# austinjeng/Shift-GCN

Measured on AMD Instinct MI355X. Metric: skeleton clips/sec fwd+bwd, NTU (3,300,25,2) bs=64; 1/2/4/8 MI355X, higher is better.
Workload: dtype fp32; 1 GPU; NTU Shift-GCN training step (fwd+CE+bwd+SGD), x=(64,3,300,25,2) per GPU; global_batch=64, per_gpu_batch=64, parallelism=dp1, hipgraph=False, world_size=1, backend=none

## Files before the change

### include/shiftgcn.h

```cpp
#ifndef SHIFTGCN_H_
#define SHIFTGCN_H_

#include <stddef.h>

#ifdef __cplusplus
extern "C" {
#endif

#define SGCN_EINVAL (-22)
#define SGCN_ABI_VERSION 25
#define SGCN_ABI_DIAG_FLAG 0x10000

int sgcn_abi_version(void);


int sgcn_tshift_fwd(const float* in, float* out, const float* xpos, const float* ypos,
                    const float* in_scale, const float* in_shift, float* plane_stats,
                    int B, int C, int H, int W, int stride, int ypos_is_raw, void* stream);

int sgcn_tshift_fwd_pre(const float* z, float* out, const float* xpos, const float* ypos,
                        const float* pre_scale, const float* pre_shift, const float* r,
                        const float* r_scale, const float* r_shift, const float* in_scale,
                        const float* in_shift, int B, int C, int H, int W, int stride,
                        int ypos_is_raw, void* stream);
// ... 92 lines not shown
                         const float* mean, const float* invstd, const float* gamma,
                         float* dgamma, float* dbeta, int accumulate, int batch_stats,
                         float* coef, void* stream);

int sgcn_bn_bwd_finalize_gbn(const float* part6, int B, int C, int V, long long n_total,
                             const float* dy_coef, const float* dy_mean, const float* mean,
                             const float* invstd, const float* gamma, float* dgamma,
                             float* dbeta, int accumulate, int batch_stats, float* coef,
                             void* stream);

int sgcn_bn_bwd_apply(const float* dy, const float* y, int relu, const float* x,
                      const float* coef, int per_joint, const float* r, const float* rcoef,
                      const float* dy_coef, float* dx, float* dr, int B, int C, int T, int V,
                      void* stream);

int sgcn_mask_prep(const float* mask, float* m, int n, void* stream);

int sgcn_gcn_gather(const float* x0, const float* m, float* xg, int B, int C, int T, int V,
                    void* stream);

#define SGCN_DXF_MASK_DX 1
#define SGCN_DXF_ADD2_PLANE 2
int sgcn_gcn_dx_finish(const float* dxt, const float* x0, const float* m, const float* add1,
                       const float* add2, const float* add2_mask, float* dx, float* dmask_part,
                       const float* prev_s, const float* prev_mean, const float* prev_invstd,
                       float* prev_part, int B, int C, int T, int V, int flags, void* stream);

int sgcn_mask_grad_finalize(const float* part, const float* mask, int B, int C, int V,
                            float* dmask, int accumulate, void* stream);

// ... 67 lines not shown
```

### shift-gcn_amd/csrc/bn.hip

```cpp
#include "common.hpp"
#include "dispatch.hpp"
#include "launch_forms.hpp"

namespace sgcn {
namespace {

constexpr int kU = 4;

constexpr int kUM = 8;

template <bool PER_JOINT, bool ZU = false>
__global__ __launch_bounds__(kThreads) void moments_kernel(const float* __restrict__ x,
                                                            float2* __restrict__ part, int T,
                                                            int V, int C) {
  SGCN_CRIT_PRIO();
  __shared__ float s1[kThreads], s2[kThreads], red[2 * kThreads / 64];
  const int plane = gridDim.x - 1 - blockIdx.x;
  const int P = T * V;
  const float* __restrict__ xp = x + (size_t)plane * P;
  const int i = threadIdx.x;
  if (PER_JOINT) {
    const int G = kThreads / V;
    float a = 0.f, q = 0.f;
    const int v = i % V, r = i / V;
// ... 730 lines not shown
  const int f = PER_JOINT ? c * V + w : c;
  const float k1 = coef[f], k2 = coef[F + f], k3 = coef[2 * F + f];
  float d1 = 1.f, d2 = 0.f, d3 = 0.f, q1 = 0.f, q2 = 0.f, q3 = 0.f;
  if (DYT) { d1 = dyc[c]; d2 = dyc[C + c]; d3 = dyc[2 * C + c]; }
  if (RES == 2) { q1 = rcoef[c]; q2 = rcoef[RF + c]; q3 = rcoef[2 * RF + c]; }
  const auto dxr = make_rsrc(dx + off, pb);
  const auto drr = make_rsrc(RES ? dr + off : dx + off, RES ? pb : 0u);
#pragma unroll
  for (int e = 0; e < LPT; ++e) {
    float g = gv[e];
    if (DYT) g = d1 * g + d2 * yv[e] + d3;
    if (RELU) g = yv[e] > 0.f ? g : 0.f;
    bstore(dxr, k1 * g + k2 * xv[e] + k3, go + e * vstep, 0);
    if (RES == 1) bstore(drr, g, vo + e * vstep, 0);
    if (RES == 2) bstore(drr, q1 * g + q2 * rv[e] + q3, vo + e * vstep, 0);
  }
}

template <int NT, int LPT, bool ADD1, bool ADD2, bool PART, int A2M>
__global__ __launch_bounds__(NT) void gcn_dx_finish_ja_kernel(
    const float* __restrict__ dxt, const float* __restrict__ x0, const float* __restrict__ m,
    const float* __restrict__ add1, const float* __restrict__ add2, float* __restrict__ dx,
    float* __restrict__ dmask_part, const float* __restrict__ ps,
    const float* __restrict__ pmean, const float* __restrict__ pinvstd,
    float2* __restrict__ bn_part, int C, int T, int V, const float* __restrict__ add2m,
    int flags) {
  SGCN_CRIT_PRIO();
  __shared__ float s0[NT];
  __shared__ float red[2 * NT / 64];
  const int plane = blockIdx.x, c = plane % C, rc = c % V;
// ... 427 lines not shown
    bn_bwd_apply_ja_kernel<NT, LPT, PJM, RL, RS, DYT><<<g, int(NT), 0, st>>>(
        dy, y, x, coef, F, r, rcoef, C, dy_coef, dx, dr, C, T, V);
  };
  auto loop = [&](auto PJM, auto RL, auto RS, auto DYT) {
    bn_bwd_apply_kernel<PJM, RL, RS, DYT><<<g, kThreads, 0, st>>>(
        dy, y, x, coef, F, r, rcoef, C, dy_coef, dx, dr, C, T, V);
  };
  const bool ok = per_joint == 3
                      ? launch_plane(T, V, ja, loop, Const<3>{}, Const<true>{}, rs, dyt)
                      : launch_plane(T, V, ja, loop, Const<0>{}, relu != 0, rs, dyt);
  SGCN_REQUIRE(ok);
  SGCN_LAUNCH_CHECK();
  return 0;
}

int sgcn_mask_prep(const float* mask, float* m, int n, void* stream) {
  SGCN_REQUIRE(mask && m && n > 0);
  mask_prep_kernel<<<(n + 255) / 256, 256, 0, (hipStream_t)stream>>>(mask, m, n);
  SGCN_LAUNCH_CHECK();
  return 0;
}

int sgcn_mask_prep_many(const float* const* mask, float* const* m, const int* count, int n,
                        void* stream) {
  SGCN_REQUIRE(n >= 0 && n <= SGCN_BATCH_MAX);
  if (n == 0) return 0;
  SGCN_REQUIRE(mask && m && count);
  MaskPrepBatch t{};
  int mx = 0;
  for (int i = 0; i < n; ++i) {
// ... 90 lines not shown
```

### shift-gcn_amd/csrc/tshift.hip

```cpp
#include "common.hpp"
#include "dispatch.hpp"
#include "launch_forms.hpp"

#pragma clang fp contract(off)

namespace sgcn {
namespace {


struct Geom {
  int x1, y1;
  float dx, dy;
};

__device__ __forceinline__ Geom make_geom(float x, float y) {
  Geom g;
  g.x1 = (int)floorf(x);
  g.y1 = (int)floorf(y);
  g.dx = x - (float)g.x1;
  g.dy = y - (float)g.y1;
  return g;
}

__device__ __forceinline__ float blend(float q11, float q21, float q12, float q22, float dx,
                                       float dy) {
  const float omdx = 1.f - dx, omdy = 1.f - dy;
  return q11 * omdx * omdy + q21 * dx * omdy + q12 * omdx * dy + q22 * dx * dy;
}

struct Walker {
  int h, w, dh, dw, W;
  __device__ __forceinline__ Walker(int o0, int step, int W_) : W(W_) {
    h = o0 / W_;
    w = o0 - h * W_;
    dh = step / W_;
    dw = step - dh * W_;
  }
  __device__ __forceinline__ void next() {
    h += dh;
    w += dw;
    if (w >= W) { w -= W; ++h; }
  }
};
// ... 204 lines not shown
          const float gg = o < nt ? gv[e] : 0.f;
          ax += vx * gg;
          ay += vy * gg;
        }
      }
    }
  }
  block_sum2(ax, ay, red);
  if (threadIdx.x == 0) pgrad[plane] = make_float2(ax, ay);
  if (BNP) {
    block_sum2(bs0, bs1, red);
    if (threadIdx.x == 0) bn_part[plane] = make_float2(bs0, bs1);
  }
}


template <int NT>
__device__ __forceinline__ void zero_pad(float* lds, int H, int W) {
  const int WP = W + 2, nprow = 2 * kPadRows * WP;
  for (int i = (int)threadIdx.x; i < nprow + 2 * H; i += NT) {
    int a;
    if (i < nprow) {
      const int r = i / WP, col = i - r * WP;
      a = (r < kPadRows ? r : H + r) * WP + col;
    } else {
      const int j = i - nprow;
      a = ((j >> 1) + kPadRows) * WP + ((j & 1) ? W + 1 : 0);
    }
    lds[a] = 0.f;
  }
}

template <int NT, int LPT, bool AFFINE>
__device__ __forceinline__ void stage_plane(const float* __restrict__ src, float* lds, int n,
                                            float a, float b) {
  float t[LPT];
#pragma unroll
  for (int e = 0; e < LPT; ++e) t[e] = src[min(e * NT + (int)threadIdx.x, n - 1)];
#pragma unroll
  for (int e = 0; e < LPT; ++e) {
    const int i = e * NT + threadIdx.x;
    if (i < n) lds[i] = AFFINE ? t[e] * a + b : t[e];
  }
}

template <int NT, int EPT, int LPT, bool AFFINE, bool STATS>
// ... 453 lines not shown
    }
  }
  if (BNP) {
    block_sum4(ax, ay, bs0, bs1, red);
    if (threadIdx.x == 0) {
      pgrad[plane] = make_float2(ax, ay);
      bn_part[plane] = make_float2(bs0, bs1);
    }
  } else {
    block_sum2(ax, ay, red);
    if (threadIdx.x == 0) pgrad[plane] = make_float2(ax, ay);
  }
}

template <int NT, int LPT, bool AFFINE, bool RELU_MASK, bool BNP, int GP, bool GBN,
          bool GBD = false>
__global__ __launch_bounds__(NT) void tshift_bwd_ra_kernel(
    const float* __restrict__ gout, const float* __restrict__ in,
    const float* __restrict__ xpos, const float* __restrict__ ypos,
    const float* __restrict__ scale, const float* __restrict__ shift,
    const float* __restrict__ bn_mean, const float* __restrict__ bn_invstd,
    float* __restrict__ gin, float2* __restrict__ pgrad, float2* __restrict__ bn_part, int C,
    int H, int W, const float* __restrict__ gdy, const float* __restrict__ gy,
    const float* __restrict__ gx, const float* __restrict__ gcoef,
    const float* __restrict__ gz, const float* __restrict__ gzm,
    const float* __restrict__ gzi, float* __restrict__ gzpart, const float* __restrict__ gd = nullptr,
    const float* __restrict__ gdm = nullptr, const float* __restrict__ gdi = nullptr,
    float* __restrict__ gdpart = nullptr, int gdyp = 0) {
  SGCN_CRIT_PRIO();
  static_assert(!GBN || (AFFINE && BNP && !GP), "GBN: shift_in with BNP");
  static_assert(!GBD || GBN, "GBD extends GBN");
  extern __shared__ float lds[];
  __shared__ float red[4 * NT / 64];
  const int plane = gridDim.x - 1 - blockIdx.x;
  const int c = plane % C;
  const int n = H * W, WP = W + 2;
  const int GR = NT / W, NTE = GR * W;
  const int tid = threadIdx.x;
  const bool own = tid < NTE;
  const int w = tid % W, h0 = tid / W;
  const unsigned vo = own ? (unsigned)tid * 4u : 0x80000000u;
  const unsigned vstep = (unsigned)NTE * 4u, nbytes = (unsigned)n * 4u;
  const size_t poff = (size_t)plane * n;
  float t[LPT], rin_r[LPT];
  float zr[GBN ? LPT : 1], dr[GBD ? LPT : 1];
  {
// ... 57 lines not shown
    lds[own && e * NTE + tid < n ? lbase + e * lstep : lspare] = t[e];
  float bmu = 0.f, bis = 0.f;
  if (BNP) { bmu = bn_mean[c]; bis = bn_invstd[c]; }
  const float x = xpos[c], y = ypos[c];
  float a = 1.f, b = 0.f;
  if (AFFINE) { a = scale[c]; b = shift[c]; }
  float zm = 0.f, zi = 0.f, dmu = 0.f, dis = 0.f;
  if (GBN) { zm = gzm[c * W + w]; zi = gzi[c * W + w]; }
  if (GBD) { dmu = gdm[c]; dis = gdi[c]; }
  __syncthreads();

  const Geom r = make_geom(-x, -y);
  const Geom g = make_geom(x, y);
  const bool fits = r.y1 >= -kPadRows && r.y1 <= kPadRows - 1 && g.y1 >= -kPadRows &&
                    g.y1 <= kPadRows - 1 && r.x1 >= -1 && r.x1 <= 0 && g.x1 >= -1 && g.x1 <= 0;
  const int kq = r.y1 * WP + r.x1, kg = (-g.y1 - 1) * WP - g.x1 - 1;
  const int nfull = n / NTE;
  const int lmax = (H - 1 + kPadRows) * WP + W;
  const auto gir = make_rsrc(gin + poff, nbytes);
  float bs0 = 0.f, bs1 = 0.f, ax = 0.f, ay = 0.f;
  float a6[6] = {0.f, 0.f, 0.f, 0.f, 0.f, 0.f};
  float d6[6] = {0.f, 0.f, 0.f, 0.f, 0.f, 0.f};
  auto elem = [&](int e, bool tail, float q11, float q21, float q12, float q22, float G11,
                  float G21, float G12, float G22) {
    const bool ok = !tail || e * NTE + tid < n;
    float val = blend(q11, q21, q12, q22, r.dx, r.dy);
    const float rin = rin_r[e];
    if (RELU_MASK) val = rin > 0.f ? val : 0.f;
    if (tail) val = ok ? val : 0.f;
    bstore(gir, val, vo + e * vstep, 0);
    if (GBN) {
      const bool act = rin > 0.f;
      const float hc = act ? rin - bmu : 0.f, zh = act ? (zr[e] - zm) * zi : 0.f;
      const float vv = act ? val : 0.f;
      a6[0] += vv;
      a6[1] += hc;
      a6[2] += act ? 1.f : 0.f;
      a6[3] = fmaf(vv, zh, a6[3]);
      a6[4] = fmaf(hc, zh, a6[4]);
      a6[5] += zh;
      if (GBD) {
        const float dh = act ? (dr[e] - dmu) * dis : 0.f;
        d6[0] += vv;
        d6[1] += hc;
        d6[2] += act ? 1.f : 0.f;
// ... 7 lines not shown
      bs1 = fmaf(val, (rin - bmu) * bis, bs1);
    }
    const float cx = (1.f - g.dy) * (G21 - G11) + g.dy * (G22 - G12);
    const float cy = (1.f - g.dx) * (G12 - G11) + g.dx * (G22 - G21);
    float qa = AFFINE ? rin * a + b : rin;
    if (tail) qa = ok ? qa : 0.f;
    ax = fmaf(qa, cx, ax);
    ay = fmaf(qa, cy, ay);
  };
  if (own && fits) {
    int l0 = lbase;
#pragma unroll
    for (int e = 0; e < LPT; ++e) {
      const bool tail = e >= nfull;
      const int lt = min(l0, lmax);
      const int la = lt + kq, lg = lt + kg;
      elem(e, tail, lds[la], lds[la + 1], lds[la + WP], lds[la + WP + 1], lds[lg + WP + 1],
           lds[lg + WP], lds[lg + 1], lds[lg]);
      l0 += lstep;
      asm volatile("" : "+v"(l0));
    }
  } else if (own) {
    const auto inr = make_rsrc(in + poff, nbytes);
    const auto zrr = make_rsrc(GBN ? gz + poff : in + poff, nbytes);
    int wz = w - c % W;
    wz = wz < 0 ? wz + W : wz;
    auto tap = [&](int row, int col) {
      const bool in_ = (unsigned)row < (unsigned)H && (unsigned)col < (unsigned)W;
      const int rr = min(max(row, 0), H - 1), cc = min(max(col, 0), W - 1);
      const float v = lds[(rr + kPadRows) * WP + cc + 1];
      return in_ ? v : 0.f;
    };
#pragma unroll 1
    for (int e = 0; e < LPT; ++e) {
      const int h = h0 + e * GR;
      const bool ok = e * NTE + tid < n;
      const float rin = bload(inr, vo + e * vstep, 0);
      const float zv = GBN ? bload(zrr, vo + e * vstep + (unsigned)((wz - w) * 4), 0) : 0.f;
      const int rq = h + r.y1, cq = w + r.x1, rg = h - g.y1 - 1, cg = w - g.x1 - 1;
      float val = blend(tap(rq, cq), tap(rq, cq + 1), tap(rq + 1, cq), tap(rq + 1, cq + 1),
                        r.dx, r.dy);
      if (RELU_MASK) val = rin > 0.f ? val : 0.f;
      val = ok ? val : 0.f;
      bstore(gir, val, vo + e * vstep, 0);
      if (GBN && rin > 0.f) {
        const float hc = rin - bmu, zh = (zv - zm) * zi;
        a6[0] += val;
        a6[1] += hc;
        a6[2] += 1.f;
        a6[3] = fmaf(val, zh, a6[3]);
        a6[4] = fmaf(hc, zh, a6[4]);
        a6[5] += zh;
        if (GBD) {
          const float dh = (bload(make_rsrc(gd + poff, nbytes), vo + e * vstep, 0) - dmu) * dis;
          d6[0] += val;
          d6[1] += hc;
          d6[2] += 1.f;
          d6[3] = fmaf(val, dh, d6[3]);
          d6[4] = fmaf(hc, dh, d6[4]);
// ... 117 lines not shown
  const float *gout, *in, *xpos, *ypos, *scale, *shift, *bmu, *bis;
  float* gin;
  float2 *pg, *bp;
  int B, C, H, W;
  const float *gdy, *gy, *gx, *gcoef;
  int gdyp;
  const float *gz, *gzm, *gzi;
  float* gzpart;
  const float *gd, *gdm, *gdi;
  float* gdpart;
};

template <const auto& Forms, class... A>
bool launch_ra(const LaunchForm& f, const RaArgs& a, hipStream_t st, A... flags) {
  return with_form<Forms>({f.nt, f.lpt}, [&](auto NT, auto LPT, auto AFFINE, auto RELU, auto BNP,
                                           auto GP, auto GBN, auto GBD) {
    tshift_bwd_ra_kernel<NT, LPT, AFFINE, RELU, BNP, GP, GBN, GBD>
        <<<a.B * a.C, int(NT), ra_lds_bytes(a.H, a.W, NT, GBN), st>>>(
            a.gout, a.in, a.xpos, a.ypos, a.scale, a.shift, a.bmu, a.bis, a.gin, a.pg, a.bp, a.C,
            a.H, a.W, a.gdy, a.gy, a.gx, a.gcoef, a.gz, a.gzm, a.gzi, a.gzpart, a.gd, a.gdm,
            a.gdi, a.gdpart, a.gdyp);
  }, flags...);
}

}
}

using namespace sgcn;

extern "C" {

int sgcn_tshift_fwd(const float* in, float* out, const float* xpos, const float* ypos,
// ... 120 lines not shown
  SGCN_REQUIRE(f.kind == Kind::ra);
  SGCN_REQUIRE(dy && s && coef && in && xpos && ypos && gin && ws);
  SGCN_REQUIRE((gx == nullptr) == (gy == nullptr));
  SGCN_REQUIRE(ws_bytes >= sgcn_tshift_bwd_ws_bytes(B, C));
  SGCN_REQUIRE((long long)B * C < (1LL << 31));
  (void)ypos_is_raw;
  hipStream_t st = (hipStream_t)stream;
  float2* pg = (float2*)ws;
  RaArgs a{nullptr, in, xpos, ypos, nullptr, nullptr, nullptr, nullptr, gin, pg, nullptr, B, C, H, W};
  a.gdy = dy;
  a.gy = y;
  a.gx = s;
  a.gcoef = coef;
  a.gdyp = dy_plane != 0;
  const bool ok = launch_ra<kBninForms>(f, a, st, Const<false>{}, Const<true>{}, Const<false>{},
                                        OneOf<1, 2>{y ? 1 : 2}, Const<false>{}, Const<false>{});
  SGCN_REQUIRE(ok);
  SGCN_LAUNCH_CHECK();
  if (gx) tshift_pos_finalize_kernel<<<(C + 3) / 4, 256, 0, st>>>(pg, B, C, gx, gy);
  SGCN_LAUNCH_CHECK();
  return 0;
}

size_t sgcn_tshift_bwd_ws_bytes(int B, int C) { return (size_t)B * C * sizeof(float2); }

int sgcn_tshift_pos_finalize_many(const void* const* partials, float* const* gx,
                                  float* const* gy, const int* B, const int* C, int n,
                                  void* stream) {
  SGCN_REQUIRE(n >= 0 && n <= SGCN_BATCH_MAX);
  if (n == 0) return 0;
  SGCN_REQUIRE(partials && gx && gy && B && C);
// ... 21 lines not shown
  return 0;
}

int sgcn_tshift_bwd_gbn(const float* gout, const float* in, const float* xpos,
                        const float* ypos, const float* in_scale, const float* in_shift,
                        const float* bn_mean, const float* bn_invstd, float* bn_part,
                        const float* z, const float* z_mean, const float* z_invstd,
                        float* z_part, const float* d, const float* d_mean,
                        const float* d_invstd, float* d_part, float* gin, float* gx, float* gy,
                        void* ws, size_t ws_bytes, int B, int C, int H, int W, void* stream) {
  SGCN_REQUIRE(B > 0 && C > 0 && H > 0 && W > 0);
  SGCN_REQUIRE((d == nullptr) == (d_part == nullptr) && (!d || (d_mean && d_invstd)));
  const LaunchForm f = gbn_form(H, W, d != nullptr);
  SGCN_REQUIRE(f.kind == Kind::ra);
  SGCN_REQUIRE(gout && in && xpos && ypos && in_scale && in_shift && bn_mean && bn_invstd &&
               bn_part && z && z_mean && z_invstd && z_part && gin && ws);
  SGCN_REQUIRE((gx == nullptr) == (gy == nullptr));
  SGCN_REQUIRE(ws_bytes >= sgcn_tshift_bwd_ws_bytes(B, C));
  SGCN_REQUIRE((long long)B * C < (1LL << 31));
  hipStream_t st = (hipStream_t)stream;
  float2* pg = (float2*)ws;
  RaArgs a{gout, in, xpos, ypos, in_scale, in_shift, bn_mean, bn_invstd, gin, pg,
           (float2*)bn_part, B, C, H, W};
  a.gz = z;
  a.gzm = z_mean;
  a.gzi = z_invstd;
  a.gzpart = z_part;
  if (d) {
    a.gd = d;
    a.gdm = d_mean;
    a.gdi = d_invstd;
    a.gdpart = d_part;
  }
  const Const<true> on{};
  const Const<false> off{};
  const bool ok = d ? launch_ra<kGbdForms>(f, a, st, on, off, on, Const<0>{}, on, on)
                    : launch_ra<kRaForms>(f, a, st, on, off, on, Const<0>{}, on, off);
  SGCN_REQUIRE(ok);
  SGCN_LAUNCH_CHECK();
  if (gx) tshift_pos_finalize_kernel<<<(C + 3) / 4, 256, 0, st>>>(pg, B, C, gx, gy);
  SGCN_LAUNCH_CHECK();
  return 0;
}

int sgcn_tshift_bwd(const float* gout, const float* in, const float* xpos, const float* ypos,
                    const float* in_scale, const float* in_shift, int relu_mask,
                    const float* bn_mean, const float* bn_invstd, float* bn_part, float* gin,
                    float* gx, float* gy, void* ws, size_t ws_bytes, int B, int C, int H,
                    int W, int stride, int ypos_is_raw, void* stream) {
  SGCN_REQUIRE(B > 0 && C > 0 && H >= 0 && W > 0 && (stride == 1 || stride == 2));
  SGCN_REQUIRE((in_scale == nullptr) == (in_shift == nullptr));
  const int Ho = H / stride;
  SGCN_REQUIRE((gout || Ho == 0) && (in || H == 0) && (gin || H == 0));
  SGCN_REQUIRE(xpos && ypos && ws && (gx == nullptr) == (gy == nullptr));
  SGCN_REQUIRE(!bn_part || (bn_mean && bn_invstd));
  SGCN_REQUIRE(ws_bytes >= sgcn_tshift_bwd_ws_bytes(B, C));
  SGCN_REQUIRE((long long)H * W < (1LL << 30) && (long long)B * C < (1LL << 31));
  hipStream_t st = (hipStream_t)stream;
  const bool aff = in_scale != nullptr, relu = relu_mask != 0, bnp = bn_part != nullptr;
  float2* pg = (float2*)ws;
  float2* bp = (float2*)bn_part;
  const int ah = (ypos_is_raw && stride != 1) ? 1 : 0;
  const LaunchForm f = bwd_form(H, W, stride);
  bool ok;
  if (f.kind == Kind::ra) {
    const RaArgs a{gout, in, xpos, ypos, in_scale, in_shift, bn_mean, bn_invstd, gin, pg, bp, B,
                   C, H, W};
    ok = launch_ra<kRaForms>(f, a, st, aff, relu, bnp, Const<0>{}, Const<false>{}, Const<false>{});
  } else if (f.kind == Kind::s2) {
    const size_t lds = (size_t)(H + Ho) * W * sizeof(float);
    ok = with_consts([&](auto LPT, auto JA, auto AFFINE, auto RELU, auto BNP) {
      tshift_bwd_s2_kernel<kBwdThreads, LPT, AFFINE, RELU, BNP, JA><<<B * C, kBwdThreads, lds, st>>>(
          gout, in, xpos, ypos, in_scale, in_shift, bn_mean, bn_invstd, gin, pg, bp, C, H, W, Ho,
          ah);
    }, OneOf<8, 16, 32>{f.lpt}, f.flag, aff, relu, bnp);
  } else {
    ok = with_consts([&](auto EPT, auto STRIDE, auto AFFINE, auto RELU, auto BNP) {
      tshift_bwd_kernel<EPT, AFFINE, RELU, STRIDE, BNP><<<B * C, kThreads, 0, st>>>(
          gout, in, xpos, ypos, in_scale, in_shift, bn_mean, bn_invstd, gin, pg, bp, C, H, W, Ho,
          ah);
    }, OneOf<8, 16, 32>{f.lpt}, OneOf<1, 2>{stride}, aff, relu, bnp);
  }
  SGCN_REQUIRE(ok);
// ... 8 lines not shown
```

### shift-gcn_amd/shiftgcn/_lib.py

```python
from __future__ import annotations

import ctypes
import os

import torch

LIB_NAME = "libshiftgcn_hip.so"
LIB_PATH = os.path.join(os.path.dirname(os.path.abspath(__file__)), LIB_NAME)
LIB_PATH = os.environ.get("SGCN_LIB_PATH", LIB_PATH)
ABI_VERSION = 25
BATCH_MAX = 32
SEQ_MAX_WM = 2048
ABI_DIAG_FLAG = 0x10000
EINVAL = -22

_lib = None

_P = ctypes.c_void_p
_I = ctypes.c_int
_F = ctypes.c_float
_Z = ctypes.c_size_t
_L = ctypes.c_longlong

SIGNATURES = {
# ... 23 lines not shown
    "sgcn_pw_dw_ws_bytes": (_Z, [_I, _I, _I, _I, _I]),
    "sgcn_pw_dw": (_I, [_P, _L, _L, _I, _I, _P, _L, _L, _I, _I, _P, _P, _I, _I, _P, _I, _P, _Z,
                        _I, _I, _I, _I, _I, _P]),
    "sgcn_moments_ws_bytes": (_Z, [_I, _I, _I, _I]),
    "sgcn_moments": (_I, [_P, _P, _I, _I, _I, _I, _I, _P]),
    "sgcn_bn_finalize": (_I, [_P, _I, _I, _I, _I, _P, _P, _F, _F, _P, _P, _P, _P, _P, _P, _P,
                              _P]),
    "sgcn_bn_eval_coef": (_I, [_I, _I, _P, _P, _P, _P, _F, _P, _P, _P, _P, _P]),
    "sgcn_bn_apply": (_I, [_P, _P, _P, _I, _P, _P, _P, _I, _P, _P, _P, _P, _I, _I, _I, _I,
                           _P]),
    "sgcn_bn_bwd_reduce": (_I, [_P, _P, _I, _P, _P, _P, _I, _P, _P, _P, _P, _P, _P, _I, _I, _I,
                                _I, _I, _P]),
    "sgcn_bn_bwd_finalize": (_I, [_P, _I, _I, _L, _I, _P, _P, _P, _P, _P, _I, _I, _P, _P]),
    "sgcn_bn_bwd_apply": (_I, [_P, _P, _I, _P, _P, _I, _P, _P, _P, _P, _P, _I, _I, _I, _I,
                               _P]),
    "sgcn_mask_prep": (_I, [_P, _P, _I, _P]),
    "sgcn_gcn_gather": (_I, [_P, _P, _P, _I, _I, _I, _I, _P]),
    "sgcn_gcn_dx_finish": (_I, [_P, _P, _P, _P, _P, _P, _P, _P, _P, _P, _P, _P, _I, _I, _I, _I,
                                _I, _P]),
    "sgcn_tshift_bwd_bnin": (_I, [_P, _P, _P, _P, _P, _P, _P, _P, _P, _P, _P, _Z, _I, _I, _I,
                                  _I, _I, _I, _P]),
    "sgcn_mask_grad_finalize": (_I, [_P, _P, _I, _I, _I, _P, _I, _P]),
    "sgcn_modalities": (_I, [_P, _P, _P, _P, _P, _P, _P, _P, _I, _I, _I, _I, _I, _I, _P]),
    "sgcn_window_normalize": (_I, [_P, _P, _P, _I, _I, _I, _I, _I, _I, _I, _I, _I, _I, _I, _I,
                                   _P]),
    "sgcn_window_aggregate": (_I, [_P, _P, _P, _I, _I, _P]),
    "sgcn_clip_augment": (_I, [_P, _P, _P, _P, _P, _P, _P, _I, _I, _I, _I, _I, _I, _I, _I, _P]),
    "sgcn_tshift_bwd_gbn": (_I, [_P, _P, _P, _P, _P, _P, _P, _P, _P, _P, _P, _P, _P, _P, _P, _P,
                                 _P, _P, _P, _P, _P, _Z, _I, _I, _I, _I, _P]),
    "sgcn_bn_bwd_finalize_gbn": (_I, [_P, _I, _I, _I, _L, _P, _P, _P, _P, _P, _P, _P, _I, _I,
# ... 63 lines not shown
```

### shift-gcn_amd/shiftgcn/fused.py

```python
from __future__ import annotations

import collections
import os
import threading

import torch

from . import ops
from .ops import PlaneView as PV


def _empty(*shape, like):
    return torch.empty(shape, device=like.device, dtype=torch.float32)


_SIDE = {}


def _side_stream(device):
    s = _SIDE.get(device)
    if s is None:
        s = _SIDE.setdefault(device, torch.cuda.Stream(device=device))
    return s

# ... 203 lines not shown
        return ops.mask_prep(fm)
    return ops.cached(gcn, "_sgcn_mask", ops._src_key((fm,)), lambda: ops.mask_prep(fm),
                      fm.device)


def prepare_masks(gcns):
    fms = [g.Feature_Mask for g in gcns]
    if any(g.training for g in gcns):
        ms = ops.mask_prep_many(fms)
    else:
        ms = ops.cached(gcns[0], "_sgcn_masks", ops._src_key(fms) + tuple(map(id, gcns)),
                        lambda: ops.mask_prep_many(fms), fms[0].device)
    return [(fm, fm._version, m) for fm, m in zip(fms, ms)]


def gcn_backward(mod, s: GcnSaved, dH, extra_dx=None, dy_coef=None, prev=None, pre6=None,
                 off=False, mask_dx=False):
    x0 = s.x0
    assert not (mask_dx and mod.has_down)
    B, Cin, T, V = x0.shape
    Cout = mod.out_channels
    g = {}
    rpart = None
    if pre6 is not None:
        assert dy_coef is not None and (pre6[2] is not None) == mod.has_down
        coefZ, g["bn.weight"], g["bn.bias"] = ops.bn_bwd_finalize_gbn(
            pre6[0], B, Cout, V, B * T, dy_coef, pre6[1], s.zst, mod.bn)
    else:
        if mod.has_down:
            conv, bnd = mod.down[0], mod.down[1]
            part, rpart = ops.bn_bwd_reduce(dH, s.H, True, s.Z, s.zst, 3, r=s.D0,
                                            rst=s.dst, dy_coef=dy_coef)
        else:
            part, rpart = ops.bn_bwd_reduce(dH, s.H, True, s.Z, s.zst, 3, dy_coef=dy_coef)
        coefZ, g["bn.weight"], g["bn.bias"] = ops.bn_bwd_finalize(part, B, Cout * V, B * T,
                                                                   s.zst, mod.bn, perm_V=V)
    dZ = _empty(B, Cout, T, V, like=x0)
    g_id = dD0 = None
    if mod.has_down:
        conv, bnd = mod.down[0], mod.down[1]
        if pre6 is not None:
            coefD, g["down.1.weight"], g["down.1.bias"] = ops.bn_bwd_finalize_gbn(
                pre6[2], B, Cout, 1, B * T * V, dy_coef, pre6[1], s.dst, bnd)
        else:
            coefD, g["down.1.weight"], g["down.1.bias"] = ops.bn_bwd_finalize(
                rpart, B, Cout, B * T * V, s.dst, bnd)
        dD0 = _empty(B, Cout, T, V, like=x0)
        ops.bn_bwd_apply(dH, s.H, True, s.Z, coefZ, 3, r=s.D0, rcoef=coefD, dr=dD0, dx=dZ,
                         dy_coef=dy_coef)
    else:
        g_id = _empty(B, Cin, T, V, like=x0)
        ops.bn_bwd_apply(dH, s.H, True, s.Z, coefZ, 3, dr=g_id, dx=dZ, dy_coef=dy_coef)
    dLW = ops.grad_like(mod.Linear_weight)
    dLb = ops.grad_like(mod.Linear_bias)
    dXt = _empty(B, Cin, T, V, like=x0)
    ops.pw_fwd(mod.Linear_weight, False, None, PV(dZ), PV(dXt), Cin, Cout, T, V)
    with _OffPath(off, dZ, s.xg):
        ops.pw_dw(PV(dZ), PV(s.xg), dLW, Cout, Cin, T, V, transpose=True, dbias=dLb)
    g["Linear_weight"], g["Linear_bias"] = _late(dLW, off), _late(dLb, off)
    a2, a2m = extra_dx or (None, None)
    res = ops.gcn_dx_finish(dXt, x0, s.m, add1=g_id, add2=a2, prev=prev, add2_mask=a2m,
                            mask_dx=mask_dx)
    dx, mpart, prev_part = res if prev is not None else (*res, None)
    dmask = ops.grad_like(mod.Feature_Mask)
    fm = mod.Feature_Mask
    if BATCH_SIDE and (off or _defer_ok((fm,))):
        _task(mpart.device).mask.append((mpart, fm, B, Cin, V, dmask))
# ... 126 lines not shown
        dRp, gx, gy = ops.tshift_bwd(dS, s.R, so.xpos.detach(), so.ypos.detach(), so.stride,
                                     relu_mask=True, defer_pos=off,
                                     pos_out=_pos_alloc(so, off))
    g["shift_out.xpos"], g["shift_out.ypos"] = _pos_grads(gx, gy, so)
    tl = mod.temporal_linear
    dWt = ops.grad_like(tl.weight)
    dbt = ops.grad_like(tl.bias)

    dAs = _empty(B, C, T, V, like=H)
    ops.pw_fwd(tl.weight, True, None, PV(dRp), PV(dAs), C, Cout, T, V)
    with _OffPath(off, dRp, s.As):
        ops.pw_dw(PV(dRp), PV(s.As), dWt, Cout, C, T, V, dbias=dbt)
    g["temporal_linear.weight"], g["temporal_linear.bias"] = _late(dWt, off), _late(dbt, off)
    if gcn_z is not None and GBN_FUSION and si.stride == 1 and ops.ra_fits(T * V, V):
        down = gcn_z[2] if len(gcn_z) > 2 else None
        res = ops.tshift_bwd_gbn(dAs, H, si.xpos.detach(), si.ypos.detach(), s.ast, gcn_z[0],
                                 gcn_z[1], defer_pos=off, down=down,
                                 pos_out=_pos_alloc(si, off))
        dA, gx, gy, part, zpart = res[:5]
        pre6 = (zpart, s.ast, res[5] if down is not None else None)
    else:
        dA, gx, gy, part = ops.tshift_bwd(
            dAs, H, si.xpos.detach(), si.ypos.detach(), si.stride, scale=s.ast.scale,
            shift=s.ast.shift, bn_stats=s.ast, defer_pos=off, pos_out=_pos_alloc(si, off))
    g["shift_in.xpos"], g["shift_in.ypos"] = _pos_grads(gx, gy, si)
    coef, g["bn.weight"], g["bn.bias"] = ops.bn_bwd_finalize(part, B, C, B * T * V, s.ast,
                                                             mod.bn)
    if not materialize_dx:
        return (dA, coef), g, pre6
    dH = ops.bn_bwd_apply(dA, None, False, H, coef, False)
    return dH, g, pre6


class ConvBnSaved:
# ... 201 lines not shown
    g.update({"tcn1." + k: v for k, v in gt.items()})
    g.update({"gcn1." + k: v for k, v in gg.items()})
    if kind == "conv":
        gr = convbn_dx_and_dw(unit.residual, s.rs, dres, dx, accumulate=True, off=off)
        g.update({"residual." + k: v for k, v in gr.items()})
    return dx, g


TSHIFT_FUSION_MIN_C = int(os.environ.get("SGCN_TSHIFT_FUSION_MIN_C", "512"))
TSHIFT_TWO_ROW = int(os.environ.get("SGCN_TSHIFT_TWO_ROW", "2"))
EVAL_FOLD = int(os.environ.get("SGCN_EVAL_FOLD", "1"))
GBN_FUSION = int(os.environ.get("SGCN_GBN_FUSION", "2"))
ASYNC_DW = int(os.environ.get("SGCN_ASYNC_DW", "1"))
PREMASK = int(os.environ.get("SGCN_PREMASK", "1"))

EVAL_PRECISIONS = ("fp32", "bf16")


def check_precision(precision):
    if precision not in EVAL_PRECISIONS:
        raise ValueError(f"eval precision must be one of {EVAL_PRECISIONS}, got {precision!r}")
    return precision


EVAL_PRECISION = check_precision(os.environ.get("SGCN_EVAL_PRECISION", "fp32"))
BF16_MIN_K = 32


class _Precision(threading.local):
    value = EVAL_PRECISION
# ... 163 lines not shown
```

### shift-gcn_amd/shiftgcn/ops.py

```python
from __future__ import annotations

import ctypes

import torch

from . import _lib

_F32 = torch.float32


def _ptr(t):
    if t is None:
        return None
    return t.data_ptr()


class LaunchTimer:

    def __init__(self, ops_filter=None, detail=False):
        self.ops_filter = ops_filter
        self.detail = detail
        self.records = []

    def begin(self, op, flops, nbytes, device):
# ... 336 lines not shown


GBN_MAX_PLANE = 16384


def ra_fits(n, V):
    if V > 64 or n > GBN_MAX_PLANE:
        return False
    if (n // V + 2 * 4) * (V + 2) + 1 > 16384:
        return False
    nt = 256 if n <= 4096 else 512
    return -(-n // ((nt // V) * V)) <= 32


def tshift_bwd_gbn(gout, inp, xpos, ypos, st: "BnStats", z, zst: "BnStats", defer_pos=False,
                   down=None, pos_out=None):
    check_input(gout, "grad_output")
    check_input(inp, "input")
    check_input(z, "z")
    if down is not None:
        check_input(down[0], "d")
    B, C, H, W = inp.shape
    lib = _lib.load()
    dev = inp.device
    gin = torch.empty_like(inp)
    nbytes = lib.sgcn_tshift_bwd_ws_bytes(B, C)
    ws = torch.empty((max(nbytes, 4) + 3) // 4, device=dev, dtype=_F32)
    gx, gy, pp = _pos_out(defer_pos, ws, B, C, dev, pos_out)
    bpart = torch.empty((B * C * 2,), device=dev, dtype=_F32)
    zpart = torch.empty((6 * B * C * W,), device=dev, dtype=_F32)
    d, dst, dpart = None, None, None
    if down is not None:
        d, dst = down
        dpart = torch.empty((6 * B * C,), device=dev, dtype=_F32)
    nb = 4 * (gout.numel() + (3 if down is None else 4) * inp.numel())
    with _timed("tshift_bwd", 0, nb, inp, ("GBND " if down is not None else "GBN ") + _shp(inp)):
        rc = lib.sgcn_tshift_bwd_gbn(_ptr(gout), _ptr(inp), _ptr(xpos), _ptr(ypos),
                                     _ptr(st.scale), _ptr(st.shift), _ptr(st.mean),
                                     _ptr(st.invstd), _ptr(bpart), _ptr(z), _ptr(zst.mean),
                                     _ptr(zst.invstd), _ptr(zpart), _ptr(d),
                                     _ptr(dst.mean if dst is not None else None),
                                     _ptr(dst.invstd if dst is not None else None),
                                     _ptr(dpart), _ptr(gin), _ptr(gx), _ptr(gy), _ptr(ws),
                                     nbytes, B, C, H, W, _stream(inp))
    _lib.check(rc, "sgcn_tshift_bwd_gbn")
    if down is not None:
        return gin, (pp if pp is not None else gx), gy, bpart, zpart, dpart
    return gin, (pp if pp is not None else gx), gy, bpart, zpart


# ... 313 lines not shown


def bn_bwd_apply(dy, y, relu, x, coef, per_joint, r=None, rcoef=None, dr=None, dx=None,
                 dy_coef=None):
    B, C, T, V = x.shape
    dx = torch.empty_like(x) if dx is None else dx
    nb = 4 * x.numel() * (3 + (y is not None) + (r is not None) + (dr is not None))
    with _timed("bn_bwd_apply", 0, nb, x, _shp(x)):
        rc = _lib.load().sgcn_bn_bwd_apply(
            _ptr(dy), _ptr(y), int(relu), _ptr(x), _ptr(coef), int(per_joint), _ptr(r),
            _ptr(rcoef), _ptr(dy_coef), _ptr(dx), _ptr(dr), B, C, T, V, _stream(x))
    _lib.check(rc, "sgcn_bn_bwd_apply")
    return dx


def mask_prep(mask):
    check_input(mask, "Feature_Mask")
    m = torch.empty_like(mask)
    with _timed("finalize", 0, 8 * mask.numel(), mask):
        rc = _lib.load().sgcn_mask_prep(_ptr(mask), _ptr(m), mask.numel(), _stream(mask))
    _lib.check(rc, "sgcn_mask_prep")
    return m


def _arr(ctype, vals):
    return (ctype * len(vals))(*vals)


def _chunks(xs):
    for i in range(0, len(xs), _lib.BATCH_MAX):
# ... 160 lines not shown
```

Measured before the change: 2056 clips/s.

## Recompute shift input-gradient inside BN backward apply instead of materializing it

The GBN temporal-shift backward kernel can now skip storing its input gradient and only produce the BN statistics sums. The downstream BN backward apply kernel recomputes the shift gradient from gout and the shift positions, staged through LDS, before applying the BN/ReLU coefficients. This removes one full-tensor write and the later re-read per block, at the cost of reloading gout and repeating the bilinear blend in a second kernel. It is enabled by default through an environment flag.

```diff
diff --git a/include/shiftgcn.h b/include/shiftgcn.h
--- a/include/shiftgcn.h
+++ b/include/shiftgcn.h
@@ -130,6 +130,11 @@
                       const float* dy_coef, float* dx, float* dr, int B, int C, int T, int V,
                       void* stream);
 
+int sgcn_bn_bwd_apply_tsh(const float* gout, const float* xpos, const float* ypos,
+                          const float* y, const float* x, const float* coef, const float* r,
+                          const float* rcoef, const float* dy_coef, float* dx, float* dr, int B,
+                          int C, int T, int V, void* stream);
+
 int sgcn_mask_prep(const float* mask, float* m, int n, void* stream);
 
 int sgcn_gcn_gather(const float* x0, const float* m, float* xg, int B, int C, int T, int V,
diff --git a/shift-gcn_amd/csrc/bn.hip b/shift-gcn_amd/csrc/bn.hip
--- a/shift-gcn_amd/csrc/bn.hip
+++ b/shift-gcn_amd/csrc/bn.hip
@@ -1,6 +1,7 @@
 #include "common.hpp"
 #include "dispatch.hpp"
 #include "launch_forms.hpp"
+#include "shift_stage.hpp"
 
 namespace sgcn {
 namespace {
@@ -768,6 +769,89 @@
     bstore(dxr, k1 * g + k2 * xv[e] + k3, go + e * vstep, 0);
     if (RES == 1) bstore(drr, g, vo + e * vstep, 0);
     if (RES == 2) bstore(drr, q1 * g + q2 * rv[e] + q3, vo + e * vstep, 0);
+  }
+}
+
+template <int NT, int LPT, int RES>
+__global__ __launch_bounds__(NT) void bn_bwd_apply_tsh_kernel(
+    const float* __restrict__ gout, const float* __restrict__ xpos,
+    const float* __restrict__ ypos, const float* __restrict__ y, const float* __restrict__ x,
+    const float* __restrict__ coef, int F, const float* __restrict__ r,
+    const float* __restrict__ rcoef, int RF, const float* __restrict__ dyc,
+    float* __restrict__ dx, float* __restrict__ dr, int C, int T, int V) {
+  SGCN_CRIT_PRIO();
+  static_assert(RES == 1 || RES == 2, "dr = g, or the down BatchNorm's input gradient");
+  extern __shared__ float lds[];
+  const int plane = blockIdx.x, c = plane % C, rc = c % V;
+  const int WP = V + 2, GR = NT / V, NTJ = GR * V, tid = threadIdx.x;
+  const bool own = tid < NTJ;
+  const int w = tid % V, h0 = tid / V;
+  const int P = T * V;
+  const size_t off = (size_t)plane * P;
+  const unsigned vo = own ? (unsigned)tid * 4u : 0x80000000u, vstep = (unsigned)NTJ * 4u;
+  const unsigned pb = (unsigned)P * 4u;
+  int wz = w - rc;
+  wz = wz < 0 ? wz + V : wz;
+  const unsigned go = vo + (unsigned)((wz - w) * 4);
+  const auto yr = make_rsrc(y + off, pb);
+  const auto xr = make_rsrc(x + off, pb);
+  const auto rr = make_rsrc(RES == 2 ? r + off : y + off, RES == 2 ? pb : 0u);
+  float yv[LPT], xv[LPT], rv[RES == 2 ? LPT : 1];
+  {
+    const auto gr = make_rsrc(gout + off, pb);
+    float t[LPT];
+#pragma unroll
+    for (int e = 0; e < LPT; ++e) t[e] = bload(gr, vo + e * vstep, 0);
+#pragma unroll
+    for (int e = 0; e < LPT; ++e) {
+      yv[e] = bload(yr, vo + e * vstep, 0);
+      xv[e] = bload(xr, go + e * vstep, 0);
+    }
+    if (RES == 2) {
+#pragma unroll
+      for (int e = 0; e < LPT; ++e) rv[e] = bload(rr, vo + e * vstep, 0);
+    }
+    zero_pad<NT>(lds, T, V);
+    const int lb = (h0 + kPadRows) * WP + w + 1, lspare = ra_pad_floats(T, V);
+#pragma unroll
+    for (int e = 0; e < LPT; ++e)
+      lds[own && e * NTJ + tid < P ? lb + e * GR * WP : lspare] = t[e];
+  }
+  const int f = c * V + w;
+  const float k1 = coef[f], k2 = coef[F + f], k3 = coef[2 * F + f];
+  const float d1 = dyc[c], d2 = dyc[C + c], d3 = dyc[2 * C + c];
+  float q1 = 0.f, q2 = 0.f, q3 = 0.f;
+  if (RES == 2) { q1 = rcoef[c]; q2 = rcoef[RF + c]; q3 = rcoef[2 * RF + c]; }
+  const Geom rg = make_geom(-xpos[c], -ypos[c]);
+  const auto dxr = make_rsrc(dx + off, pb);
+  const auto drr = make_rsrc(dr + off, pb);
+  __syncthreads();
+  if (!own) return;
+  const int lmax = (T - 1 + kPadRows) * WP + V;
+  if (shift_in_grad_fits(rg)) {
+    int l0 = (h0 + kPadRows) * WP + w + 1;
+#pragma unroll
+    for (int e = 0; e < LPT; ++e) {
+      float g = shift_in_grad<true>(lds, rg, min(l0, lmax), 0, w, T, V);
+      g = d1 * g + d2 * yv[e] + d3;
+      g = yv[e] > 0.f ? g : 0.f;
+      bstore(dxr, k1 * g + k2 * xv[e] + k3, go + e * vstep, 0);
+      if (RES == 1) bstore(drr, g, vo + e * vstep, 0);
+      if (RES == 2) bstore(drr, q1 * g + q2 * rv[e] + q3, vo + e * vstep, 0);
+      l0 += GR * WP;
+      asm volatile("" : "+v"(l0));
+    }
+  } else {
+#pragma unroll 1
+    for (int e = 0; e < LPT; ++e) {
+      const float yy = bload(yr, vo + e * vstep, 0), xx = bload(xr, go + e * vstep, 0);
+      float g = shift_in_grad<false>(lds, rg, 0, h0 + e * GR, w, T, V);
+      g = d1 * g + d2 * yy + d3;
+      g = yy > 0.f ? g : 0.f;
+      bstore(dxr, k1 * g + k2 * xx + k3, go + e * vstep, 0);
+      if (RES == 1) bstore(drr, g, vo + e * vstep, 0);
+      if (RES == 2) bstore(drr, q1 * g + q2 * bload(rr, vo + e * vstep, 0) + q3, vo + e * vstep, 0);
+    }
   }
 }
 
@@ -1225,6 +1309,29 @@
   return 0;
 }
 
+int sgcn_bn_bwd_apply_tsh(const float* gout, const float* xpos, const float* ypos,
+                          const float* y, const float* x, const float* coef, const float* r,
+                          const float* rcoef, const float* dy_coef, float* dx, float* dr, int B,
+                          int C, int T, int V, void* stream) {
+  SGCN_REQUIRE(B > 0 && C > 0 && T > 0 && V > 0);
+  SGCN_REQUIRE(gout && xpos && ypos && y && x && coef && dy_coef && dx && dr);
+  SGCN_REQUIRE((r == nullptr) == (rcoef == nullptr));
+  SGCN_REQUIRE((long long)B * C < (1LL << 31));
+  const LaunchForm f = gbn_form(T, V, r != nullptr);
+  SGCN_REQUIRE(f.kind == Kind::ra);
+  hipStream_t st = (hipStream_t)stream;
+  const size_t lds = ra_lds_bytes(T, V, f.nt, false);
+  auto go = [&](auto NT, auto LPT, auto RES) {
+    bn_bwd_apply_tsh_kernel<NT, LPT, RES><<<B * C, int(NT), lds, st>>>(
+        gout, xpos, ypos, y, x, coef, C * V, r, rcoef, C, dy_coef, dx, dr, C, T, V);
+  };
+  const bool ok = r ? with_form<kGbdForms>({f.nt, f.lpt}, go, Const<2>{})
+                    : with_form<kRaForms>({f.nt, f.lpt}, go, Const<1>{});
+  SGCN_REQUIRE(ok);
+  SGCN_LAUNCH_CHECK();
+  return 0;
+}
+
 int sgcn_mask_prep(const float* mask, float* m, int n, void* stream) {
   SGCN_REQUIRE(mask && m && n > 0);
   mask_prep_kernel<<<(n + 255) / 256, 256, 0, (hipStream_t)stream>>>(mask, m, n);
diff --git a/shift-gcn_amd/csrc/shift_stage.hpp b/shift-gcn_amd/csrc/shift_stage.hpp
--- /dev/null
+++ b/shift-gcn_amd/csrc/shift_stage.hpp
@@ -0,0 +1,67 @@
+#pragma once
+#include "common.hpp"
+#include "launch_forms.hpp"
+
+namespace sgcn {
+
+struct Geom {
+  int x1, y1;
+  float dx, dy;
+};
+
+__device__ __forceinline__ Geom make_geom(float x, float y) {
+#pragma clang fp contract(off)
+  Geom g;
+  g.x1 = (int)floorf(x);
+  g.y1 = (int)floorf(y);
+  g.dx = x - (float)g.x1;
+  g.dy = y - (float)g.y1;
+  return g;
+}
+
+__device__ __forceinline__ float blend(float q11, float q21, float q12, float q22, float dx,
+                                       float dy) {
+#pragma clang fp contract(off)
+  const float omdx = 1.f - dx, omdy = 1.f - dy;
+  return q11 * omdx * omdy + q21 * dx * omdy + q12 * omdx * dy + q22 * dx * dy;
+}
+
+template <int NT>
+__device__ __forceinline__ void zero_pad(float* lds, int H, int W) {
+  const int WP = W + 2, nprow = 2 * kPadRows * WP;
+  for (int i = (int)threadIdx.x; i < nprow + 2 * H; i += NT) {
+    int a;
+    if (i < nprow) {
+      const int r = i / WP, col = i - r * WP;
+      a = (r < kPadRows ? r : H + r) * WP + col;
+    } else {
+      const int j = i - nprow;
+      a = ((j >> 1) + kPadRows) * WP + ((j & 1) ? W + 1 : 0);
+    }
+    lds[a] = 0.f;
+  }
+}
+
+__device__ __forceinline__ bool shift_in_grad_fits(const Geom& r) {
+  return r.y1 >= -kPadRows && r.y1 <= kPadRows - 1 && r.x1 >= -1 && r.x1 <= 0;
+}
+
+template <bool FITS>
+__device__ __forceinline__ float shift_in_grad(const float* lds, const Geom& r, int lt, int h,
+                                               int w, int H, int W) {
+  const int WP = W + 2;
+  if (FITS) {
+    const int la = lt + r.y1 * WP + r.x1;
+    return blend(lds[la], lds[la + 1], lds[la + WP], lds[la + WP + 1], r.dx, r.dy);
+  }
+  auto tap = [&](int row, int col) {
+    const bool in_ = (unsigned)row < (unsigned)H && (unsigned)col < (unsigned)W;
+    const int rr = min(max(row, 0), H - 1), cc = min(max(col, 0), W - 1);
+    const float v = lds[(rr + kPadRows) * WP + cc + 1];
+    return in_ ? v : 0.f;
+  };
+  const int rq = h + r.y1, cq = w + r.x1;
+  return blend(tap(rq, cq), tap(rq, cq + 1), tap(rq + 1, cq), tap(rq + 1, cq + 1), r.dx, r.dy);
+}
+
+}
diff --git a/shift-gcn_amd/csrc/tshift.hip b/shift-gcn_amd/csrc/tshift.hip
--- a/shift-gcn_amd/csrc/tshift.hip
+++ b/shift-gcn_amd/csrc/tshift.hip
@@ -1,6 +1,7 @@
 #include "common.hpp"
 #include "dispatch.hpp"
 #include "launch_forms.hpp"
+#include "shift_stage.hpp"
 
 #pragma clang fp contract(off)
 
@@ -8,25 +9,6 @@
 namespace {
 
 
-struct Geom {
-  int x1, y1;
-  float dx, dy;
-};
-
-__device__ __forceinline__ Geom make_geom(float x, float y) {
-  Geom g;
-  g.x1 = (int)floorf(x);
-  g.y1 = (int)floorf(y);
-  g.dx = x - (float)g.x1;
-  g.dy = y - (float)g.y1;
-  return g;
-}
-
-__device__ __forceinline__ float blend(float q11, float q21, float q12, float q22, float dx,
-                                       float dy) {
-  const float omdx = 1.f - dx, omdy = 1.f - dy;
-  return q11 * omdx * omdy + q21 * dx * omdy + q12 * omdx * dy + q22 * dx * dy;
-}
 
 struct Walker {
   int h, w, dh, dw, W;
@@ -261,22 +243,6 @@
   }
 }
 
-
-template <int NT>
-__device__ __forceinline__ void zero_pad(float* lds, int H, int W) {
-  const int WP = W + 2, nprow = 2 * kPadRows * WP;
-  for (int i = (int)threadIdx.x; i < nprow + 2 * H; i += NT) {
-    int a;
-    if (i < nprow) {
-      const int r = i / WP, col = i - r * WP;
-      a = (r < kPadRows ? r : H + r) * WP + col;
-    } else {
-      const int j = i - nprow;
-      a = ((j >> 1) + kPadRows) * WP + ((j & 1) ? W + 1 : 0);
-    }
-    lds[a] = 0.f;
-  }
-}
 
 template <int NT, int LPT, bool AFFINE>
 __device__ __forceinline__ void stage_plane(const float* __restrict__ src, float* lds, int n,
@@ -760,7 +726,7 @@
 }
 
 template <int NT, int LPT, bool AFFINE, bool RELU_MASK, bool BNP, int GP, bool GBN,
-          bool GBD = false>
+          bool GBD = false, bool STORE = true>
 __global__ __launch_bounds__(NT) void tshift_bwd_ra_kernel(
     const float* __restrict__ gout, const float* __restrict__ in,
     const float* __restrict__ xpos, const float* __restrict__ ypos,
@@ -776,6 +742,7 @@
   SGCN_CRIT_PRIO();
   static_assert(!GBN || (AFFINE && BNP && !GP), "GBN: shift_in with BNP");
   static_assert(!GBD || GBN, "GBD extends GBN");
+  static_assert(STORE || GBN, "sums only: the GBN forms");
   extern __shared__ float lds[];
   __shared__ float red[4 * NT / 64];
   const int plane = gridDim.x - 1 - blockIdx.x;
@@ -863,21 +830,19 @@
   const Geom g = make_geom(x, y);
   const bool fits = r.y1 >= -kPadRows && r.y1 <= kPadRows - 1 && g.y1 >= -kPadRows &&
                     g.y1 <= kPadRows - 1 && r.x1 >= -1 && r.x1 <= 0 && g.x1 >= -1 && g.x1 <= 0;
-  const int kq = r.y1 * WP + r.x1, kg = (-g.y1 - 1) * WP - g.x1 - 1;
+  const int kg = (-g.y1 - 1) * WP - g.x1 - 1;
   const int nfull = n / NTE;
   const int lmax = (H - 1 + kPadRows) * WP + W;
   const auto gir = make_rsrc(gin + poff, nbytes);
   float bs0 = 0.f, bs1 = 0.f, ax = 0.f, ay = 0.f;
   float a6[6] = {0.f, 0.f, 0.f, 0.f, 0.f, 0.f};
   float d6[6] = {0.f, 0.f, 0.f, 0.f, 0.f, 0.f};
-  auto elem = [&](int e, bool tail, float q11, float q21, float q12, float q22, float G11,
-                  float G21, float G12, float G22) {
+  auto elem = [&](int e, bool tail, float val, float G11, float G21, float G12, float G22) {
     const bool ok = !tail || e * NTE + tid < n;
-    float val = blend(q11, q21, q12, q22, r.dx, r.dy);
     const float rin = rin_r[e];
     if (RELU_MASK) val = rin > 0.f ? val : 0.f;
     if (tail) val = ok ? val : 0.f;
-    bstore(gir, val, vo + e * vstep, 0);
+    if (STORE) bstore(gir, val, vo + e * vstep, 0);
     if (GBN) {
       const bool act = rin > 0.f;
       const float hc = act ? rin - bmu : 0.f, zh = act ? (zr[e] - zm) * zi : 0.f;
@@ -915,9 +880,9 @@
     for (int e = 0; e < LPT; ++e) {
       const bool tail = e >= nfull;
       const int lt = min(l0, lmax);
-      const int la = lt + kq, lg = lt + kg;
-      elem(e, tail, lds[la], lds[la + 1], lds[la + WP], lds[la + WP + 1], lds[lg + WP + 1],
-           lds[lg + WP], lds[lg + 1], lds[lg]);
+      const int lg = lt + kg;
+      elem(e, tail, shift_in_grad<true>(lds, r, lt, 0, w, H, W), lds[lg + WP + 1], lds[lg + WP],
+           lds[lg + 1], lds[lg]);
       l0 += lstep;
       asm volatile("" : "+v"(l0));
     }
@@ -938,12 +903,11 @@
       const bool ok = e * NTE + tid < n;
       const float rin = bload(inr, vo + e * vstep, 0);
       const float zv = GBN ? bload(zrr, vo + e * vstep + (unsigned)((wz - w) * 4), 0) : 0.f;
-      const int rq = h + r.y1, cq = w + r.x1, rg = h - g.y1 - 1, cg = w - g.x1 - 1;
-      float val = blend(tap(rq, cq), tap(rq, cq + 1), tap(rq + 1, cq), tap(rq + 1, cq + 1),
-                        r.dx, r.dy);
+      const int rg = h - g.y1 - 1, cg = w - g.x1 - 1;
+      float val = shift_in_grad<false>(lds, r, 0, h, w, H, W);
       if (RELU_MASK) val = rin > 0.f ? val : 0.f;
       val = ok ? val : 0.f;
-      bstore(gir, val, vo + e * vstep, 0);
+      if (STORE) bstore(gir, val, vo + e * vstep, 0);
       if (GBN && rin > 0.f) {
         const float hc = rin - bmu, zh = (zv - zm) * zi;
         a6[0] += val;
@@ -1091,8 +1055,8 @@
 template <const auto& Forms, class... A>
 bool launch_ra(const LaunchForm& f, const RaArgs& a, hipStream_t st, A... flags) {
   return with_form<Forms>({f.nt, f.lpt}, [&](auto NT, auto LPT, auto AFFINE, auto RELU, auto BNP,
-                                           auto GP, auto GBN, auto GBD) {
-    tshift_bwd_ra_kernel<NT, LPT, AFFINE, RELU, BNP, GP, GBN, GBD>
+                                           auto GP, auto GBN, auto GBD, auto STORE) {
+    tshift_bwd_ra_kernel<NT, LPT, AFFINE, RELU, BNP, GP, GBN, GBD, STORE>
         <<<a.B * a.C, int(NT), ra_lds_bytes(a.H, a.W, NT, GBN), st>>>(
             a.gout, a.in, a.xpos, a.ypos, a.scale, a.shift, a.bmu, a.bis, a.gin, a.pg, a.bp, a.C,
             a.H, a.W, a.gdy, a.gy, a.gx, a.gcoef, a.gz, a.gzm, a.gzi, a.gzpart, a.gd, a.gdm,
@@ -1243,7 +1207,8 @@
   a.gcoef = coef;
   a.gdyp = dy_plane != 0;
   const bool ok = launch_ra<kBninForms>(f, a, st, Const<false>{}, Const<true>{}, Const<false>{},
-                                        OneOf<1, 2>{y ? 1 : 2}, Const<false>{}, Const<false>{});
+                                        OneOf<1, 2>{y ? 1 : 2}, Const<false>{}, Const<false>{},
+                                        Const<true>{});
   SGCN_REQUIRE(ok);
   SGCN_LAUNCH_CHECK();
   if (gx) tshift_pos_finalize_kernel<<<(C + 3) / 4, 256, 0, st>>>(pg, B, C, gx, gy);
@@ -1295,7 +1260,7 @@
   const LaunchForm f = gbn_form(H, W, d != nullptr);
   SGCN_REQUIRE(f.kind == Kind::ra);
   SGCN_REQUIRE(gout && in && xpos && ypos && in_scale && in_shift && bn_mean && bn_invstd &&
-               bn_part && z && z_mean && z_invstd && z_part && gin && ws);
+               bn_part && z && z_mean && z_invstd && z_part && ws);
   SGCN_REQUIRE((gx == nullptr) == (gy == nullptr));
   SGCN_REQUIRE(ws_bytes >= sgcn_tshift_bwd_ws_bytes(B, C));
   SGCN_REQUIRE((long long)B * C < (1LL << 31));
@@ -1315,8 +1280,9 @@
   }
   const Const<true> on{};
   const Const<false> off{};
-  const bool ok = d ? launch_ra<kGbdForms>(f, a, st, on, off, on, Const<0>{}, on, on)
-                    : launch_ra<kRaForms>(f, a, st, on, off, on, Const<0>{}, on, off);
+  const bool store = gin != nullptr;
+  const bool ok = d ? launch_ra<kGbdForms>(f, a, st, on, off, on, Const<0>{}, on, on, store)
+                    : launch_ra<kRaForms>(f, a, st, on, off, on, Const<0>{}, on, off, store);
   SGCN_REQUIRE(ok);
   SGCN_LAUNCH_CHECK();
   if (gx) tshift_pos_finalize_kernel<<<(C + 3) / 4, 256, 0, st>>>(pg, B, C, gx, gy);
@@ -1347,7 +1313,8 @@
   if (f.kind == Kind::ra) {
     const RaArgs a{gout, in, xpos, ypos, in_scale, in_shift, bn_mean, bn_invstd, gin, pg, bp, B,
                    C, H, W};
-    ok = launch_ra<kRaForms>(f, a, st, aff, relu, bnp, Const<0>{}, Const<false>{}, Const<false>{});
+    ok = launch_ra<kRaForms>(f, a, st, aff, relu, bnp, Const<0>{}, Const<false>{}, Const<false>{},
+                             Const<true>{});
   } else if (f.kind == Kind::s2) {
     const size_t lds = (size_t)(H + Ho) * W * sizeof(float);
     ok = with_consts([&](auto LPT, auto JA, auto AFFINE, auto RELU, auto BNP) {
diff --git a/shift-gcn_amd/shiftgcn/_lib.py b/shift-gcn_amd/shiftgcn/_lib.py
--- a/shift-gcn_amd/shiftgcn/_lib.py
+++ b/shift-gcn_amd/shiftgcn/_lib.py
@@ -61,6 +61,8 @@
     "sgcn_bn_bwd_finalize": (_I, [_P, _I, _I, _L, _I, _P, _P, _P, _P, _P, _I, _I, _P, _P]),
     "sgcn_bn_bwd_apply": (_I, [_P, _P, _I, _P, _P, _I, _P, _P, _P, _P, _P, _I, _I, _I, _I,
                                _P]),
+    "sgcn_bn_bwd_apply_tsh": (_I, [_P, _P, _P, _P, _P, _P, _P, _P, _P, _P, _P, _I, _I, _I, _I,
+                                   _P]),
     "sgcn_mask_prep": (_I, [_P, _P, _I, _P]),
     "sgcn_gcn_gather": (_I, [_P, _P, _P, _I, _I, _I, _I, _P]),
     "sgcn_gcn_dx_finish": (_I, [_P, _P, _P, _P, _P, _P, _P, _P, _P, _P, _P, _P, _I, _I, _I, _I,
diff --git a/shift-gcn_amd/shiftgcn/fused.py b/shift-gcn_amd/shiftgcn/fused.py
--- a/shift-gcn_amd/shiftgcn/fused.py
+++ b/shift-gcn_amd/shiftgcn/fused.py
@@ -241,6 +241,14 @@
     return [(fm, fm._version, m) for fm, m in zip(fms, ms)]
 
 
+class ShiftGrad:
+
+    __slots__ = ("gout", "xpos", "ypos")
+
+    def __init__(self, gout, xpos, ypos):
+        self.gout, self.xpos, self.ypos = gout, xpos, ypos
+
+
 def gcn_backward(mod, s: GcnSaved, dH, extra_dx=None, dy_coef=None, prev=None, pre6=None,
                  off=False, mask_dx=False):
     x0 = s.x0
@@ -249,6 +257,8 @@
     Cout = mod.out_channels
     g = {}
     rpart = None
+    reform = isinstance(dH, ShiftGrad)
+    assert not reform or pre6 is not None
     if pre6 is not None:
         assert dy_coef is not None and (pre6[2] is not None) == mod.has_down
         coefZ, g["bn.weight"], g["bn.bias"] = ops.bn_bwd_finalize_gbn(
@@ -273,11 +283,19 @@
             coefD, g["down.1.weight"], g["down.1.bias"] = ops.bn_bwd_finalize(
                 rpart, B, Cout, B * T * V, s.dst, bnd)
         dD0 = _empty(B, Cout, T, V, like=x0)
-        ops.bn_bwd_apply(dH, s.H, True, s.Z, coefZ, 3, r=s.D0, rcoef=coefD, dr=dD0, dx=dZ,
-                         dy_coef=dy_coef)
+        if reform:
+            ops.bn_bwd_apply_tsh(dH.gout, dH.xpos, dH.ypos, s.H, s.Z, coefZ, dy_coef, r=s.D0,
+                                 rcoef=coefD, dr=dD0, dx=dZ)
+        else:
+            ops.bn_bwd_apply(dH, s.H, True, s.Z, coefZ, 3, r=s.D0, rcoef=coefD, dr=dD0, dx=dZ,
+                             dy_coef=dy_coef)
     else:
         g_id = _empty(B, Cin, T, V, like=x0)
-        ops.bn_bwd_apply(dH, s.H, True, s.Z, coefZ, 3, dr=g_id, dx=dZ, dy_coef=dy_coef)
+        if reform:
+            ops.bn_bwd_apply_tsh(dH.gout, dH.xpos, dH.ypos, s.H, s.Z, coefZ, dy_coef, dr=g_id,
+                                 dx=dZ)
+        else:
+            ops.bn_bwd_apply(dH, s.H, True, s.Z, coefZ, 3, dr=g_id, dx=dZ, dy_coef=dy_coef)
     dLW = ops.grad_like(mod.Linear_weight)
     dLb = ops.grad_like(mod.Linear_bias)
     dXt = _empty(B, Cin, T, V, like=x0)
@@ -434,10 +452,13 @@
     g["temporal_linear.weight"], g["temporal_linear.bias"] = _late(dWt, off), _late(dbt, off)
     if gcn_z is not None and GBN_FUSION and si.stride == 1 and ops.ra_fits(T * V, V):
         down = gcn_z[2] if len(gcn_z) > 2 else None
+        reform = bool(DA_REFORM) and not materialize_dx
         res = ops.tshift_bwd_gbn(dAs, H, si.xpos.detach(), si.ypos.detach(), s.ast, gcn_z[0],
                                  gcn_z[1], defer_pos=off, down=down,
-                                 pos_out=_pos_alloc(si, off))
+                                 pos_out=_pos_alloc(si, off), store=not reform)
         dA, gx, gy, part, zpart = res[:5]
+        if reform:
+            dA = ShiftGrad(dAs, si.xpos.detach(), si.ypos.detach())
         pre6 = (zpart, s.ast, res[5] if down is not None else None)
     else:
         dA, gx, gy, part = ops.tshift_bwd(
@@ -669,6 +690,8 @@
 ASYNC_DW = int(os.environ.get("SGCN_ASYNC_DW", "1"))
 PREMASK = int(os.environ.get("SGCN_PREMASK", "1"))
 
+DA_REFORM = int(os.environ.get("SGCN_DA_REFORM", "1"))
+
 EVAL_PRECISIONS = ("fp32", "bf16")
 
 
diff --git a/shift-gcn_amd/shiftgcn/ops.py b/shift-gcn_amd/shiftgcn/ops.py
--- a/shift-gcn_amd/shiftgcn/ops.py
+++ b/shift-gcn_amd/shiftgcn/ops.py
@@ -374,7 +374,7 @@
 
 
 def tshift_bwd_gbn(gout, inp, xpos, ypos, st: "BnStats", z, zst: "BnStats", defer_pos=False,
-                   down=None, pos_out=None):
+                   down=None, pos_out=None, store=True):
     check_input(gout, "grad_output")
     check_input(inp, "input")
     check_input(z, "z")
@@ -383,7 +383,7 @@
     B, C, H, W = inp.shape
     lib = _lib.load()
     dev = inp.device
-    gin = torch.empty_like(inp)
+    gin = torch.empty_like(inp) if store else None
     nbytes = lib.sgcn_tshift_bwd_ws_bytes(B, C)
     ws = torch.empty((max(nbytes, 4) + 3) // 4, device=dev, dtype=_F32)
     gx, gy, pp = _pos_out(defer_pos, ws, B, C, dev, pos_out)
@@ -393,7 +393,7 @@
     if down is not None:
         d, dst = down
         dpart = torch.empty((6 * B * C,), device=dev, dtype=_F32)
-    nb = 4 * (gout.numel() + (3 if down is None else 4) * inp.numel())
+    nb = 4 * (gout.numel() + (2 + (down is not None) + bool(store)) * inp.numel())
     with _timed("tshift_bwd", 0, nb, inp, ("GBND " if down is not None else "GBN ") + _shp(inp)):
         rc = lib.sgcn_tshift_bwd_gbn(_ptr(gout), _ptr(inp), _ptr(xpos), _ptr(ypos),
                                      _ptr(st.scale), _ptr(st.shift), _ptr(st.mean),
@@ -737,6 +737,25 @@
     return dx
 
 
+def bn_bwd_apply_tsh(gout, xpos, ypos, y, x, coef, dy_coef, r=None, rcoef=None, dr=None,
+                     dx=None):
+    for t, n in ((gout, "grad_output"), (y, "y"), (x, "x"), (coef, "coef"),
+                 (dy_coef, "dy_coef")):
+        check_input(t, n)
+    if (r is None) != (rcoef is None):
+        raise ValueError("r and rcoef go together")
+    B, C, T, V = x.shape
+    dx = torch.empty_like(x) if dx is None else dx
+    dr = torch.empty_like(x) if dr is None else dr
+    nb = 4 * x.numel() * (5 + (r is not None))
+    with _timed("bn_bwd_apply", 0, nb, x, "TSH " + _shp(x)):
+        rc = _lib.load().sgcn_bn_bwd_apply_tsh(
+            _ptr(gout), _ptr(xpos), _ptr(ypos), _ptr(y), _ptr(x), _ptr(coef), _ptr(r),
+            _ptr(rcoef), _ptr(dy_coef), _ptr(dx), _ptr(dr), B, C, T, V, _stream(x))
+    _lib.check(rc, "sgcn_bn_bwd_apply_tsh")
+    return dx, dr
+
+
 def mask_prep(mask):
     check_input(mask, "Feature_Mask")
     m = torch.empty_like(mask)
```

Measured after the change: 2081 clips/s, median of 6. +1.2%, better.
